# JosephCatrambone/aruco3

Hardware: AMD Instinct MI355X
Metric: frames/sec at 1920x1080 ARUCO dict (higher is better)
Workload: dtype u8

## Files before the change

aruco3_amd/_lib.py:

```python
import ctypes as C
from pathlib import Path

import numpy as np

import os

_HERE = Path(__file__).resolve().parent
LIB_PATH = Path(os.environ["A3_HIP_LIB"]).resolve() if os.environ.get("A3_HIP_LIB") else _HERE / "libaruco3_hip.so"

OK, ERR_INVALID, ERR_HIP, ERR_CAPACITY, ERR_INTERNAL, ERR_NO_DEVICE, ERR_LIMIT = 0, -1, -2, -3, -4, -5, -6
FMT_RGB8, FMT_RGBA8, FMT_L8, FMT_BGRA8 = 0, 1, 2, 3
MEM_HOST, MEM_DEVICE = 0, 1
PROFILE_OFF, PROFILE_STAGES, PROFILE_THRESHOLD_ONLY, PROFILE_THRESHOLD_SAMPLED = 0, 1, 2, 3
STAGE_THRESHOLD, STAGE_CONTOUR, STAGE_DECODE = 0, 1, 2
STEP_WHOLE, STEP_DECODE_DEFERRED, STEP_HELD_RELEASED_BY_LAST, STEP_HELD_RELEASED_EARLY, STEP_BURST_LAST, STEP_HELD = 0, 1, 2, 3, 4, 5
REFINE_NONE, REFINE_SUBPIX = 0, 1
BOARD_NONE, BOARD_OK = 0, 1
BOARD_MAX_MARKERS = 1024
DIST_NONE, DIST_RATIONAL = 0, 1
DIST_FISHEYE = 3
CHARUCO_MAX_CORNERS = 2048
CHARUCO_NO_ADJ = 0xFFFFFFFF
CALIB_FIX_PRINCIPAL_POINT, CALIB_ZERO_TANGENT_DIST, CALIB_FIX_K3, CALIB_RATIONAL_MODEL, CALIB_USE_INTRINSIC_GUESS = 1, 2, 4, 8, 16
CALIB_OK, CALIB_TOO_FEW, CALIB_NO_INIT, CALIB_NOT_FINITE = 1, 2, 3, 4
# ... 6 lines not shown
RIG_OBS_USED, RIG_OBS_TOO_FEW_POINTS, RIG_OBS_DEGENERATE = 1, 2, 3
RIG_FRAME_USED, RIG_FRAME_UNUSED = 1, 2
RIG_MAX_CAMERAS, RIG_MAX_FRAMES, RIG_MAX_RIGS, RIG_MAX_CALL_FRAMES, RIG_MAX_CALL_OBSERVATIONS = 8, 4096, 1024, 65536, 262144
HANDEYE_USE_GUESS, HANDEYE_FIX_X = 1, 2
HANDEYE_OK, HANDEYE_TOO_FEW_FRAMES, HANDEYE_NO_MOTION, HANDEYE_NOT_FINITE = 1, 2, 3, 4
HANDEYE_FRAME_USED, HANDEYE_FRAME_TOO_FEW_POINTS, HANDEYE_FRAME_DEGENERATE = 1, 2, 3
HANDEYE_MAX_FRAMES, HANDEYE_MAX_PROBLEMS, HANDEYE_MAX_CALL_FRAMES = 256, 1024, 65536
HANDEYE_MIN_PIVOT_RATIO = 1e-4
MAP_USE_GUESS, MAP_FIX_MAP = 1, 2
MAP_OK, MAP_NOT_CONNECTED, MAP_NOT_FINITE = 1, 2, 3
MAP_MARKER_USED, MAP_MARKER_UNSEEN, MAP_MARKER_UNREACHED = 1, 2, 3
MAP_FRAME_USED, MAP_FRAME_UNUSED = 1, 2
MAP_OBS_USED, MAP_OBS_DEGENERATE, MAP_OBS_UNREACHED = 1, 2, 3
MAP_MAX_MARKERS, MAP_MAX_FRAMES, MAP_MAX_MAPS, MAP_MAX_CALL_FRAMES, MAP_MAX_CALL_OBSERVATIONS, MAP_START_OBSERVATIONS = 128, 4096, 1024, 65536, 262144, 8
STEP_NAMES = {0: "whole", 1: "decode_deferred", 2: "held_released_by_last", 3: "held_released_early", 4: "burst_last", 5: "held"}

SYMBOLS = [
    "a3_abi_version", "a3_default_config", "a3_create", "a3_destroy", "a3_last_error", "a3_set_stream", "a3_get_stream", "a3_set_pool_limits",
    "a3_get_tau", "a3_order_after", "a3_set_debug_taps", "a3_detect_batch", "a3_detect_batch_pose", "a3_detect_batch_submit", "a3_detect_batch_collect", "a3_detect_batch_pose_submit", "a3_detect_batch_pose_collect",
    "a3_host_alloc", "a3_host_free", "a3_host_register", "a3_host_unregister", "a3_get_stats", "a3_synth_render", "a3_download_grey", "a3_download_thresholded",
    "a3_candidate_count", "a3_download_candidates", "a3_download_homographies", "a3_estimate_pose", "a3_estimate_pose_normalized",
    "a3_find_nearest", "a3_calculate_tau", "a3_set_profiling", "a3_get_profile",
    "a3_contour_count", "a3_download_contours", "a3_detection_record_bytes", "a3_pack_detections",
    "a3_default_refine_config", "a3_set_corner_refinement", "a3_get_refined_corners", "a3_refine_corners",
    "a3_set_board", "a3_get_board_poses", "a3_estimate_board_pose",
    "a3_default_recover_config", "a3_set_board_recovery", "a3_get_board_recovery", "a3_get_recovered_counts", "a3_recover_markers",
    "a3_default_distortion", "a3_set_distortion", "a3_get_undistorted_corners", "a3_undistort_points",
    "a3_default_charuco_config", "a3_set_charuco", "a3_get_charuco_corners", "a3_get_charuco_poses", "a3_interpolate_charuco",
    "a3_calibrate_cameras", "a3_calibrate_fisheye_cameras", "a3_calibrate_rigs", "a3_calibrate_hand_eyes", "a3_build_marker_maps",
    "a3_default_rectify", "a3_rectify_frames", "a3_set_rectification", "a3_get_rectification",
]
CAND_DTYPE = np.dtype([("start_key", "<u4"), ("xy", "<u2", (8,))])
PROJ_DTYPE = np.dtype([("inv", "<f4", (9,)), ("ok", "<i4")])
INTERNAL_SYMBOLS = ["a3_debug_set_overlap", "a3_debug_build_flags", "a3_debug_spin", "a3_debug_set_hold", "a3_debug_set_jump_rounds", "a3_debug_launch_threshold", "a3_debug_kernel_time", "a3_selftest_ieee", "a3_debug_clockwise", "a3_debug_rotate_bits", "a3_debug_discard_too_near", "a3_debug_inject_candidates", "a3_debug_sample_frames", "a3_debug_frame_candidates"]


class A3Error(RuntimeError):
    def __init__(self, code, message):
        super().__init__(f"aruco3_hip error {code}: {message}")
        self.code = code


class Config(C.Structure):
    _fields_ = [
        ("threshold_window", C.c_uint32),
        ("contour_simplification_epsilon", C.c_double),
        ("min_side_length_factor", C.c_float),
        ("min_corner_separation_factor", C.c_float),
        ("homography_sample_size", C.c_uint32),
        ("filter_high_bit_errors", C.c_uint8),
    ]


class MarkerRec(C.Structure):
    _fields_ = [
        ("frame", C.c_uint32),
        ("id", C.c_uint32),
        ("code", C.c_uint64),
        ("corners", C.c_uint32 * 8),
        ("hamming_distance", C.c_uint8),
        ("rotation", C.c_uint8),
        ("candidate_index", C.c_uint16),
    ]


MARKER_DTYPE = np.dtype([("frame", "<u4"), ("id", "<u4"), ("code", "<u8"), ("corners", "<u4", (8,)), ("hamming_distance", "u1"),
                         ("rotation", "u1"), ("candidate_index", "<u2")], align=True)
# ... 359 lines not shown
        L.a3_calibrate_hand_eyes.restype = C.c_int
        L.a3_calibrate_hand_eyes.argtypes = [vp, C.POINTER(HandEyeProblem), C.c_size_t, C.POINTER(HandEyeFrame), C.c_size_t, f32p, f32p,
                                             C.POINTER(HandEyeResult), C.POINTER(HandEyeFrameResult)]
    if hasattr(L, "a3_build_marker_maps"):
        L.a3_build_marker_maps.restype = C.c_int
        L.a3_build_marker_maps.argtypes = [vp, C.POINTER(Map), C.c_size_t, C.POINTER(MapMarker), C.c_size_t, C.POINTER(MapObservation),
                                           C.c_size_t, f32p, C.POINTER(MapResult), C.POINTER(MapMarkerResult), C.POINTER(MapFrame),
                                           C.POINTER(MapObservationResult)]
    if hasattr(L, "a3_calibrate_cameras"):
        L.a3_calibrate_cameras.restype = C.c_int
        L.a3_calibrate_cameras.argtypes = [vp, C.POINTER(CalibCamera), C.c_size_t, u32p, C.c_size_t, f32p, f32p, C.POINTER(CalibResult),
                                           C.POINTER(CalibView)]
    if hasattr(L, "a3_calibrate_fisheye_cameras"):
        L.a3_calibrate_fisheye_cameras.restype = C.c_int
        L.a3_calibrate_fisheye_cameras.argtypes = [vp, C.POINTER(CalibCamera), C.c_size_t, u32p, C.c_size_t, f32p, f32p, C.POINTER(CalibResult),
                                                   C.POINTER(CalibView)]
    if hasattr(L, "a3_rectify_frames"):
        L.a3_default_rectify.restype = None
        L.a3_default_rectify.argtypes = [C.POINTER(RectifyRec), C.POINTER(Intrinsics), C.POINTER(DistortionRec)]
        L.a3_rectify_frames.restype = C.c_int
        L.a3_rectify_frames.argtypes = [vp, vp, C.c_int, C.c_int, C.c_size_t, C.c_size_t, C.c_uint32, C.POINTER(RectifyRec), vp, C.c_int,
                                        C.c_size_t, C.c_size_t, C.POINTER(RectifyInfo)]
    if hasattr(L, "a3_set_rectification"):
        L.a3_set_rectification.restype = C.c_int
        L.a3_set_rectification.argtypes = [vp, C.POINTER(RectifyRec)]
        L.a3_get_rectification.restype = C.c_int
        L.a3_get_rectification.argtypes = [vp, C.POINTER(RectifyRec), C.POINTER(C.c_int)]
    L.a3_debug_discard_too_near.restype = C.c_int
    L.a3_debug_discard_too_near.argtypes = [vp, u32p, C.c_size_t, C.c_float, u32p, C.POINTER(C.c_size_t)]
    if hasattr(L, "a3_debug_frame_candidates"):
        L.a3_debug_frame_candidates.restype = C.c_int
        L.a3_debug_frame_candidates.argtypes = [vp, C.c_uint32, C.c_uint32, u32p, vp, C.c_float, C.c_uint32, C.POINTER(C.c_uint16),
                                                C.POINTER(C.c_uint16), u32p, u32p, u32p, vp]
    _lib = L
    return L


def library_info() -> dict:
    L = load()
    flags = int(L.a3_debug_build_flags()) if hasattr(L, "a3_debug_build_flags") else -1
    return {"path": str(LIB_PATH), "from_A3_HIP_LIB": bool(os.environ.get("A3_HIP_LIB")), "tuning_build": bool(flags & 1) if flags >= 0 else None,
            "non_default_kernel_build": bool(flags & 2) if flags >= 0 else None, "abi": int(L.a3_abi_version())}


class PinnedBuffer:

    def __init__(self, nbytes: int):
        p = C.c_void_p()
        rc = load().a3_host_alloc(nbytes, C.byref(p))
        if rc != OK:
            raise A3Error(rc, load().a3_last_error(None).decode("utf-8", "replace"))
        self.ptr, self.nbytes = p.value, nbytes
        self.array = np.ctypeslib.as_array((C.c_uint8 * nbytes).from_address(p.value))

    def close(self):
        if getattr(self, "ptr", None):
            self.array = None
            load().a3_host_free(C.c_void_p(self.ptr))
            self.ptr = None

    def __del__(self):
        try:
            self.close()
        except Exception:
            pass

# ... 456 lines not shown
    def debug_inject_candidates(self, quads: np.ndarray):
        q = np.ascontiguousarray(quads, dtype=np.uint32).reshape(-1, 8)
        check(load().a3_debug_inject_candidates(self.handle, _p(q, C.c_uint32), q.shape[0]), self)

    def debug_sample_frames(self, on: bool):
        check(load().a3_debug_sample_frames(self.handle, int(on)), self.handle)

    def debug_discard_too_near(self, quads: np.ndarray, min_distance: float) -> np.ndarray:
        q = np.ascontiguousarray(quads, dtype=np.uint32).reshape(-1, 8)
        out = np.zeros_like(q)
        n = C.c_size_t()
        check(load().a3_debug_discard_too_near(self.handle, _p(q, C.c_uint32), q.shape[0], min_distance, _p(out, C.c_uint32), C.byref(n)),
              self.handle)
        return out[: n.value].reshape(-1, 4, 2)

    def debug_frame_candidates(self, cand_count, records: np.ndarray, max_cand: int, min_distance: float, S: int = 0) -> dict:
        cnt = np.ascontiguousarray(cand_count, dtype=np.uint32).reshape(-1)
        rec = np.ascontiguousarray(records, dtype=CAND_DTYPE).reshape(-1)
        n = cnt.shape[0]
        if max_cand >= 1 and rec.shape[0] != int(np.minimum(cnt, max_cand).sum()):
            raise ValueError("records must hold min(cand_count, max_cand) entries per frame")
        slots = n * max_cand if 1 <= max_cand <= 65536 else 0
        pre = np.empty((n, slots // max(n, 1), 8), dtype=np.uint16)
        fin = np.empty_like(pre)
        fin_count = np.empty(n, dtype=np.uint32)
        work = np.empty(slots, dtype=np.uint32)
        work_count = np.zeros(1, dtype=np.uint32)
        proj = np.empty(slots if S else 0, dtype=PROJ_DTYPE)
        check(load().a3_debug_frame_candidates(self.handle, n, max_cand, _p(cnt, C.c_uint32), rec.ctypes.data if rec.size else None, min_distance, S,
                                               _p(pre, C.c_uint16), _p(fin, C.c_uint16), _p(fin_count, C.c_uint32), _p(work, C.c_uint32),
                                               _p(work_count, C.c_uint32), proj.ctypes.data if S else None), self.handle)
        return {"pre_xy": pre, "fin_xy": fin, "fin_count": fin_count, "work": work, "work_count": int(work_count[0]), "proj": proj if S else None}

    def estimate_pose(self, corners: np.ndarray, marker_size_mm: float, image_size=None, intrinsics: Intrinsics = None) -> np.ndarray:
        c = np.ascontiguousarray(corners, dtype=np.uint32).reshape(-1, 8)
        out = (PoseRec * (2 * max(c.shape[0], 1)))()
        iw, ih = image_size if image_size else (1, 1)
        check(load().a3_estimate_pose(self.handle, _p(c, C.c_uint32), c.shape[0], marker_size_mm, C.byref(intrinsics) if intrinsics else None,
                                      iw, ih, out), self.handle)
        return out

    def estimate_pose_normalized(self, points: np.ndarray, marker_size_mm: float):
        p = np.ascontiguousarray(points, dtype=np.float32).reshape(-1, 8)
        out = (PoseRec * (2 * max(p.shape[0], 1)))()
        check(load().a3_estimate_pose_normalized(self.handle, _p(p, C.c_float), p.shape[0], marker_size_mm, out), self.handle)
        return out

    def find_nearest(self, bits: np.ndarray):
        b = np.ascontiguousarray(bits, dtype=np.uint64)
        idx = np.zeros(max(b.size, 1), dtype=np.uint32)
        dist = np.zeros(max(b.size, 1), dtype=np.uint8)
        check(load().a3_find_nearest(self.handle, _p(b, C.c_uint64), b.size, _p(idx, C.c_uint32), _p(dist, C.c_uint8)), self.handle)
        return idx[: b.size], dist[: b.size]

    def selftest_ieee(self, a: np.ndarray, b: np.ndarray):
        a = np.ascontiguousarray(a, dtype=np.float64)
        b = np.ascontiguousarray(b, dtype=np.float64)
        n = a.size
        sq, dv = np.zeros(n), np.zeros(n)
        sqf, dvf = np.zeros(n, dtype=np.float32), np.zeros(n, dtype=np.float32)
        check(load().a3_selftest_ieee(self.handle, _p(a, C.c_double), _p(b, C.c_double), n, _p(sq, C.c_double), _p(dv, C.c_double),
                                      _p(sqf, C.c_float), _p(dvf, C.c_float)), self.handle)
        return sq, dv, sqf, dvf


_dict_ctx = {}
# ... 22 lines not shown
```

aruco3_amd/csrc/a3_api.hip:

```cpp
#include <algorithm>
#include <atomic>
#include <cmath>
#include <chrono>
#include <cstddef>
#include <cstdio>
#include <cstring>
#include <mutex>
#include <string>
#include <vector>

#include "a3_common.h"
#include "a3_internal.h"
#include "a3_launch.h"
#include "a3_readback.h"
#include "a3_rectify_check.h"
#include "a3_solve_check.h"

using namespace a3;

namespace {

thread_local std::string g_create_error;

constexpr uint32_t kPatchCapMin = 32768, kPatchCapMax = 1u << 20;
// ... 1790 lines not shown
    if (int rcs_ = need_stream(ctx)) return rcs_;
    struct Own : DevBuf { ~Own() { release(); } } d_cands, d_cnt, d_pre, d_fin, d_work, d_proj, d_big;
    const bool big = max_cand > frame_cand_lds_slots();
    const size_t proj_bytes = S ? slots * proj_rec_bytes() : 0;
    A3_HIP(d_cands.ensure(slots * sizeof(CandRec)));
    A3_HIP(d_cnt.ensure(((size_t)2 * n_frames + 1) * 4));
    A3_HIP(d_pre.ensure(slots * 16)); A3_HIP(d_fin.ensure(slots * 16)); A3_HIP(d_work.ensure(slots * 4));
    if (S) A3_HIP(d_proj.ensure(proj_bytes));
    if (big) A3_HIP(d_big.ensure(slots * 4));
    uint32_t* cnt = d_cnt.as<uint32_t>();
    hipStream_t st = ctx->stream;
    A3_HIP(hipMemcpyAsync(d_cands.p, h.data(), slots * sizeof(CandRec), hipMemcpyHostToDevice, st));
    A3_HIP(hipMemcpyAsync(cnt, cand_count, (size_t)n_frames * 4, hipMemcpyHostToDevice, st));
    A3_HIP(hipMemsetAsync(cnt + n_frames, 0xFF, (size_t)n_frames * 4, st));
    A3_HIP(hipMemsetAsync(cnt + 2 * (size_t)n_frames, 0, 4, st));
    A3_HIP(hipMemsetAsync(d_pre.p, 0xFF, slots * 16, st)); A3_HIP(hipMemsetAsync(d_fin.p, 0xFF, slots * 16, st));
    A3_HIP(hipMemsetAsync(d_work.p, 0xFF, slots * 4, st));
    if (S) A3_HIP(hipMemsetAsync(d_proj.p, 0xFF, proj_bytes, st));
    if (big) A3_HIP(hipMemsetAsync(d_big.p, 0xFF, slots * 4, st));
    A3_HIP(launch_frame_candidates(st, {.n_frames = n_frames, .max_cand = max_cand, .cands = d_cands.as<CandRec>(), .cand_count = cnt, .min_distance = min_distance,
                                        .pre_xy = d_pre.as<uint16_t>(), .fin_xy = d_fin.as<uint16_t>(), .fin_count = cnt + n_frames, .work = d_work.as<uint32_t>(),
                                        .work_count = cnt + 2 * (size_t)n_frames, .S = S, .proj = S ? d_proj.p : nullptr,
                                        .big_scratch = big ? d_big.as<float>() : nullptr}));
    A3_HIP(hipMemcpyAsync(pre_xy, d_pre.p, slots * 16, hipMemcpyDeviceToHost, st));
    A3_HIP(hipMemcpyAsync(fin_xy, d_fin.p, slots * 16, hipMemcpyDeviceToHost, st));
    A3_HIP(hipMemcpyAsync(fin_count, cnt + n_frames, (size_t)n_frames * 4, hipMemcpyDeviceToHost, st));
    A3_HIP(hipMemcpyAsync(work, d_work.p, slots * 4, hipMemcpyDeviceToHost, st));
    A3_HIP(hipMemcpyAsync(work_count, cnt + 2 * (size_t)n_frames, 4, hipMemcpyDeviceToHost, st));
    if (S) A3_HIP(hipMemcpyAsync(proj, d_proj.p, proj_bytes, hipMemcpyDeviceToHost, st));
    A3_HIP(hipStreamSynchronize(ctx->stream));
    return A3_OK;
}

int a3_debug_inject_candidates(a3_ctx* ctx, const uint32_t* quads_xy, size_t n) {
    if (!ctx || (!quads_xy && n)) return A3_ERR_INVALID;
    if (ctx->batch.active || ctx->pending_trivial) return fail(ctx, A3_ERR_INVALID, "a3_debug_inject_candidates: a submitted batch has not been collected");
    if (n > kMaxCandDefault) return fail(ctx, A3_ERR_CAPACITY, "a3_debug_inject_candidates: at most 1024 quads");
    ctx->inject.resize(n);
    for (size_t i = 0; i < n; i++) {
        ctx->inject[i].start_key = (uint32_t)i;
        for (int k = 0; k < 8; k++) {
            if (quads_xy[8 * i + k] > 65535u) return fail(ctx, A3_ERR_INVALID, "coordinates above 65535");
            ctx->inject[i].xy[k] = (uint16_t)quads_xy[8 * i + k];
        }
    }
    ctx->inject_armed = true;
    return A3_OK;
}

int a3_debug_sample_frames(a3_ctx* ctx, int enabled) {
    if (!ctx) return A3_ERR_INVALID;
    ctx->debug_sample_frames = enabled != 0;
    return A3_OK;
}

void a3_default_refine_config(a3_refine_config* cfg) {
    if (!cfg) return;
    cfg->method = A3_REFINE_SUBPIX; cfg->win_half = 5; cfg->relative_win = 0.4f; cfg->max_iterations = 30; cfg->min_shift = 0.01f;
}

static int check_refine_config(a3_ctx* ctx, const a3_refine_config& c) {
    if (c.method != A3_REFINE_NONE && c.method != A3_REFINE_SUBPIX) return fail(ctx, A3_ERR_INVALID, "a3_refine_config.method: unknown method");
    if (c.method == A3_REFINE_NONE) return A3_OK;
    if (c.win_half < 1 || c.win_half > 10) return fail(ctx, A3_ERR_INVALID, "a3_refine_config.win_half must be in 1..10");
    if (!(c.relative_win >= 0.0f) || !std::isfinite(c.relative_win)) return fail(ctx, A3_ERR_INVALID, "a3_refine_config.relative_win must be finite and >= 0");
    if (c.max_iterations > 100) return fail(ctx, A3_ERR_INVALID, "a3_refine_config.max_iterations must be at most 100");
// ... 690 lines not shown
```

aruco3_amd/csrc/a3_internal.h:

```cpp
#ifndef ARUCO3_HIP_INTERNAL_H
#define ARUCO3_HIP_INTERNAL_H

#include "../../include/aruco3_hip.h"

#ifdef __cplusplus
extern "C" {
#endif

int  a3_debug_kernel_time(a3_ctx *ctx, int kernel, int dbg, int reps, float *avg_ms);

int  a3_debug_set_overlap(int mode);

int  a3_debug_spin(void *hip_stream, int workgroups, int threads, int usec);

int  a3_debug_set_hold(int on);

int  a3_debug_set_jump_rounds(int rounds);

int  a3_debug_launch_threshold(a3_ctx *ctx, const void *pixels_device, int fmt, uint32_t width, uint32_t height, uint32_t n_frames);

int  a3_debug_build_flags(void);

int  a3_selftest_ieee(a3_ctx *ctx, const double *a, const double *b, size_t n, double *sqrt_a, double *a_div_b,
                      float *sqrtf_a, float *a_divf_b);

int  a3_debug_clockwise(a3_ctx *ctx, const int32_t *quads_xy, size_t n, int32_t *out_xy);
int  a3_debug_rotate_bits(a3_ctx *ctx, const uint8_t *bits, uint32_t n, uint32_t times, uint8_t *out);
int  a3_debug_inject_candidates(a3_ctx *ctx, const uint32_t *quads_xy, size_t n);
int  a3_debug_sample_frames(a3_ctx *ctx, int enabled);
int  a3_debug_discard_too_near(a3_ctx *ctx, const uint32_t *quads_xy, size_t n, float min_distance, uint32_t *out_xy, size_t *n_out);

typedef struct { uint32_t start_key; uint16_t xy[8]; } a3_debug_cand;
#define A3_DEBUG_PROJ_BYTES 40
int  a3_debug_frame_candidates(a3_ctx *ctx, uint32_t n_frames, uint32_t max_cand, const uint32_t *cand_count, const a3_debug_cand *records,
                               float min_distance, uint32_t S, uint16_t *pre_xy, uint16_t *fin_xy, uint32_t *fin_count, uint32_t *work,
                               uint32_t *work_count, void *proj);

#ifdef __cplusplus
}
#endif
#endif
```

aruco3_amd/csrc/k_contours.hip:

```cpp
#include <algorithm>
#include <cmath>

#include "a3_common.h"
#include "a3_launch.h"


namespace a3 {

constexpr int kFinB = 8;
constexpr int kScatB = 1;

struct Nb8 { uint64_t c; uint64_t n[8]; };

__device__ __forceinline__ uint64_t ldw(const uint64_t* __restrict__ img, int wpr, int H, int j, int y) {
    return (y >= 0 && y < H && j >= 0 && j < wpr) ? img[(size_t)y * wpr + j] : 0ull;
}

__device__ __forceinline__ void pdart_words(const Nb8& nb, uint64_t p[8]) {
#pragma unroll
    for (int k = 0; k < 8; k++) {
        uint64_t m = nb.c & nb.n[k] & ~nb.n[(k + 7) & 7];
        if ((k & 1) == 0) m &= ~nb.n[(k + 6) & 7];
        p[k] = m;
    }
// ... 1324 lines not shown
    const int dx1 = hq[2] - hq[0], dy1 = hq[3] - hq[1], dx2 = hq[4] - hq[0], dy2 = hq[5] - hq[1];
    if (dx1 * dy2 - dy1 * dx2 < 0) { const int tx = hq[2], ty = hq[3]; hq[2] = hq[6]; hq[3] = hq[7]; hq[6] = tx; hq[7] = ty; }
}

__global__ void k_debug_clockwise(const int32_t* __restrict__ in, uint32_t n, int32_t* __restrict__ out) {
    const uint32_t i = blockIdx.x * blockDim.x + threadIdx.x;
    if (i >= n) return;
    int q[8];
    for (int k = 0; k < 8; k++) q[k] = in[8 * i + k];
    enforce_clockwise(q);
    for (int k = 0; k < 8; k++) out[8 * i + k] = q[k];
}

#define A3_DPP_MAX64(V, CTRL, ROWMASK)                                                                                   \
    {                                                                                                                    \
        const uint32_t lo_ = (uint32_t)__builtin_amdgcn_update_dpp(0, (int)(uint32_t)(V), CTRL, ROWMASK, 0xF, false);        \
        const uint32_t hi_ = (uint32_t)__builtin_amdgcn_update_dpp(0, (int)(uint32_t)((V) >> 32), CTRL, ROWMASK, 0xF, false); \
        const unsigned long long o_ = ((unsigned long long)hi_ << 32) | lo_;                                             \
        (V) = o_ > (V) ? o_ : (V);                                                                                       \
    }
template <int G>
__device__ __forceinline__ unsigned long long group_max_u64(unsigned long long v) {
    A3_DPP_MAX64(v, 0x111, 0xF)
    A3_DPP_MAX64(v, 0x112, 0xF)
    A3_DPP_MAX64(v, 0x114, 0xF)
    A3_DPP_MAX64(v, 0x118, 0xF)
    if constexpr (G == 16) return __shfl(v, 15, 16);
    A3_DPP_MAX64(v, 0x142, 0xA)
    A3_DPP_MAX64(v, 0x143, 0xC)
    const uint32_t lo = (uint32_t)__builtin_amdgcn_readlane((int)(uint32_t)v, 63), hi = (uint32_t)__builtin_amdgcn_readlane((int)(uint32_t)(v >> 32), 63);
    return ((unsigned long long)hi << 32) | lo;
}
#undef A3_DPP_MAX64

constexpr uint32_t kSmallBorder = 64;
template <int G>
__device__ __forceinline__ void contour_quads_body(uint32_t block, uint32_t n_blocks, const ContourRec* __restrict__ contours, const DeviceCounters* __restrict__ ctr,
                                                       uint32_t max_contours, const uint32_t* __restrict__ points, double eps_factor,
                                                       uint32_t min_edge_length, uint32_t first_frame, uint32_t max_cand,
                                                       CandRec* __restrict__ cands, uint32_t* __restrict__ cand_count,
                                                       unsigned int* __restrict__ err_flags, bool coords14) {
    if (ctr->err_flags & (kErrPointPool | kErrContourTable)) return;
    const uint32_t n_contours = min(ctr->contours, max_contours);
    const int lane = threadIdx.x & (G - 1);
    const uint32_t wave_global = (block * blockDim.x + threadIdx.x) / G, n_waves = (n_blocks * blockDim.x) / G;
    for (uint32_t c = wave_global; c < n_contours; c += n_waves) {
        const ContourRec r = contours[c];
        if ((r.n <= kSmallBorder) != (G == 16)) continue;
        const uint32_t* P = points + r.point_base;
        const uint32_t n = r.n;
        const double eps = (double)n * eps_factor;
        uint32_t seg_a[8], seg_b[8];
        int nseg = 1, splits = 0;
        uint32_t kept[3];
        seg_a[0] = 0; seg_b[0] = n - 1;
        bool reject = false;
        while (nseg > 0 && !reject) {
            nseg--;
            const uint32_t a = seg_a[nseg], b = seg_b[nseg];
            const uint32_t pa = P[a], pb = P[b];
            const int ax = pa & 0xFFFF, ay = pa >> 16, bx = pb & 0xFFFF, by = pb >> 16;
            const int la = ay - by, lb = bx - ax;
            const long long lc = (long long)ax * by - (long long)bx * ay;
            unsigned long long best = 0;
            for (uint32_t i0 = a + 1 + lane; i0 <= b; i0 += 4 * G) {
                uint32_t p[4];
#pragma unroll
                for (int u = 0; u < 4; u++) p[u] = P[min(i0 + (uint32_t)u * G, b)];
#pragma unroll
                for (int u = 0; u < 4; u++) {
                    const uint32_t i = i0 + (uint32_t)u * G;
                    if (i > b) break;
                    unsigned long long anum;
                    if (coords14) {
                        const int v = __mul24(la, (int)(p[u] & 0xFFFF)) + __mul24(lb, (int)(p[u] >> 16)) + (int)lc;
                        anum = (unsigned long long)(uint32_t)(v < 0 ? -v : v);
                    } else {
                        long long num = (long long)la * (int)(p[u] & 0xFFFF) + (long long)lb * (int)(p[u] >> 16) + lc;
                        anum = (unsigned long long)(num < 0 ? -num : num);
                    }
                    const unsigned long long cand = (anum << 30) | (unsigned long long)(~i & 0x3FFFFFFFu);
                    if (cand > best) best = cand;
                }
            }
            best = group_max_u64<G>(best);
            const unsigned long long num = best >> 30;
            if (num == 0) continue;
            const uint32_t index = ~(uint32_t)best & 0x3FFFFFFFu;
            const double dn = (double)num, den = (double)((long long)la * la + (long long)lb * lb);
            const double lhs = dn * dn, rhs = eps * eps * den;
            bool far;
            if (lhs > rhs * (1.0 + 1e-9)) far = true;
            else if (lhs < rhs * (1.0 - 1e-9)) far = false;
            else far = dn / sqrt(den) > eps;
            if (far) {
                if (splits == 3) { reject = true; break; }
                kept[splits++] = index;
                seg_a[nseg] = a; seg_b[nseg] = index; nseg++;
                seg_a[nseg] = index; seg_b[nseg] = b; nseg++;
            }
        }
        if (reject || splits != 3) continue;
        if (lane != 0) continue;
        uint32_t k0 = kept[0], k1 = kept[1], k2 = kept[2], t;
        if (k0 > k1) { t = k0; k0 = k1; k1 = t; }
        if (k1 > k2) { t = k1; k1 = k2; k2 = t; }
        if (k0 > k1) { t = k0; k0 = k1; k1 = t; }
        const uint32_t idx[4] = {0u, k0, k1, k2};
        int q[8], hq[8];
        for (int i = 0; i < 4; i++) { const uint32_t p = P[idx[i]]; q[2 * i] = p & 0xFFFF; q[2 * i + 1] = p >> 16; }
        if (!hull4(q, hq)) continue;
        uint32_t cmin = min_edge_length + 1u;
        for (int i = 0; i < 4; i++) {
            const int j = (i + 1) & 3;
            const int dx = hq[2 * i] - hq[2 * j], dy = hq[2 * i + 1] - hq[2 * j + 1];
            const uint32_t d2 = (uint32_t)(dx * dx + dy * dy);
            cmin = d2 < cmin ? d2 : cmin;
        }
        if (cmin < min_edge_length) continue;
        enforce_clockwise(hq);
        const uint32_t fl = r.frame - first_frame;
        const uint32_t slot = atomicAdd(&cand_count[fl], 1u);
        if (slot >= max_cand) { atomicOr(err_flags, kErrCandTable); continue; }
        CandRec cr;
        cr.start_key = r.start_key;
        for (int i = 0; i < 8; i++) cr.xy[i] = (uint16_t)hq[i];
        cands[(size_t)fl * max_cand + slot] = cr;
    }
}

__global__ __launch_bounds__(256) void k_contour_quads(uint32_t blocks64, const ContourRec* __restrict__ contours, const DeviceCounters* __restrict__ ctr,
                                                       uint32_t max_contours, const uint32_t* __restrict__ points, double eps_factor,
                                                       uint32_t min_edge_length, uint32_t first_frame, uint32_t max_cand,
                                                       CandRec* __restrict__ cands, uint32_t* __restrict__ cand_count,
                                                       unsigned int* __restrict__ err_flags, int coords14) {
    if (blockIdx.x < blocks64)
        contour_quads_body<64>(blockIdx.x, blocks64, contours, ctr, max_contours, points, eps_factor, min_edge_length, first_frame, max_cand, cands,
                               cand_count, err_flags, coords14 != 0);
    else
        contour_quads_body<16>(blockIdx.x - blocks64, gridDim.x - blocks64, contours, ctr, max_contours, points, eps_factor, min_edge_length,
                               first_frame, max_cand, cands, cand_count, err_flags, coords14 != 0);
}

__global__ void k_unpack_bits(const uint64_t* __restrict__ bits, int W, int H, uint8_t* __restrict__ out) {
    const int x = blockIdx.x * blockDim.x + threadIdx.x, y = blockIdx.y;
    if (x >= W) return;
    const int wpr = (int)words_per_row((uint32_t)W);
    out[(size_t)y * W + x] = ((bits[(size_t)y * wpr + (x >> 6)] >> (x & 63)) & 1ull) ? 255 : 0;
}

constexpr int kFinBlocks = 1536;
static inline int blocks_for(uint64_t n, int per_block, int cap) {
    uint64_t b = (n + per_block - 1) / per_block;
    if (b < 1) b = 1;
    if (b > (uint64_t)cap) b = cap;
    return (int)b;
}

__global__ __launch_bounds__(256) void k_zero(uint4* __restrict__ p, uint32_t n16) {
    for (uint32_t i = blockIdx.x * blockDim.x + threadIdx.x; i < n16; i += gridDim.x * blockDim.x) p[i] = make_uint4(0u, 0u, 0u, 0u);
}
hipError_t launch_zero(hipStream_t st, void* p, size_t bytes) {
    const uint32_t n16 = (uint32_t)(bytes / 16);
    hipLaunchKernelGGL(k_zero, dim3(blocks_for(n16, 256, 256)), dim3(256), 0, st, reinterpret_cast<uint4*>(p), n16);
    return hipGetLastError();
}

static size_t tile_off_offset(uint32_t W, uint32_t H, uint32_t n_frames) { return (size_t)dart_tiles(W, H) * n_frames; }
static size_t tile_mask_offset_bytes(uint32_t W, uint32_t H, uint32_t n_frames) { return ((size_t)dart_tiles(W, H) * n_frames * 4 * (1 + kCountHalves) + 7) & ~(size_t)7; }
size_t tile_darts_bytes(uint32_t W, uint32_t H, uint32_t n_frames) { return tile_mask_offset_bytes(W, H, n_frames) + (size_t)dart_tiles(W, H) * n_frames * kCountHalves * 8; }

hipError_t launch_dart_count(hipStream_t st, const DartCountLaunch& d) {
    const uint64_t* const bits = d.bits; const int W = d.W, H = d.H; const uint32_t first_frame = d.first_frame, n_frames = d.n_frames;
    unsigned long long* const frame_darts = d.frame_darts; uint32_t* const tile_darts = d.tile_darts; PlanWords* const plan = d.plan;
// ... 139 lines not shown
```

Measured before the change: 382,800.

## Stage contour points in LDS and use packed dot for Douglas-Peucker quad fitting

```diff
diff --git a/aruco3_amd/_lib.py b/aruco3_amd/_lib.py
--- a/aruco3_amd/_lib.py
+++ b/aruco3_amd/_lib.py
@@ -62,7 +62,7 @@
 ]
 CAND_DTYPE = np.dtype([("start_key", "<u4"), ("xy", "<u2", (8,))])
 PROJ_DTYPE = np.dtype([("inv", "<f4", (9,)), ("ok", "<i4")])
-INTERNAL_SYMBOLS = ["a3_debug_set_overlap", "a3_debug_build_flags", "a3_debug_spin", "a3_debug_set_hold", "a3_debug_set_jump_rounds", "a3_debug_launch_threshold", "a3_debug_kernel_time", "a3_selftest_ieee", "a3_debug_clockwise", "a3_debug_rotate_bits", "a3_debug_discard_too_near", "a3_debug_inject_candidates", "a3_debug_sample_frames", "a3_debug_frame_candidates"]
+INTERNAL_SYMBOLS = ["a3_debug_set_overlap", "a3_debug_build_flags", "a3_debug_spin", "a3_debug_set_hold", "a3_debug_set_jump_rounds", "a3_debug_launch_threshold", "a3_debug_kernel_time", "a3_selftest_ieee", "a3_debug_clockwise", "a3_debug_rotate_bits", "a3_debug_discard_too_near", "a3_debug_inject_candidates", "a3_debug_sample_frames", "a3_debug_frame_candidates", "a3_debug_contour_quads"]
 
 
 class A3Error(RuntimeError):
@@ -488,6 +488,10 @@
         L.a3_debug_frame_candidates.restype = C.c_int
         L.a3_debug_frame_candidates.argtypes = [vp, C.c_uint32, C.c_uint32, u32p, vp, C.c_float, C.c_uint32, C.POINTER(C.c_uint16),
                                                 C.POINTER(C.c_uint16), u32p, u32p, u32p, vp]
+    if hasattr(L, "a3_debug_contour_quads"):
+        L.a3_debug_contour_quads.restype = C.c_int
+        L.a3_debug_contour_quads.argtypes = [vp, C.c_uint32, C.c_uint32, C.c_uint32, u32p, u32p, u32p, C.c_double, C.c_uint32, C.c_uint32,
+                                             u32p, vp, u32p]
     _lib = L
     return L
 
@@ -1010,6 +1014,24 @@
                                                _p(work_count, C.c_uint32), proj.ctypes.data if S else None), self.handle)
         return {"pre_xy": pre, "fin_xy": fin, "fin_count": fin_count, "work": work, "work_count": int(work_count[0]), "proj": proj if S else None}
 
+    def debug_contour_quads(self, size, borders, eps_factor: float, min_edge_length: int, max_cand: int = 1024) -> dict:
+        per_frame = np.array([len(f) for f in borders], dtype=np.uint32)
+        flat = [np.asarray(b, dtype=np.int64).reshape(-1, 2) for f in borders for b in f]
+        lengths = np.array([b.shape[0] for b in flat], dtype=np.uint32)
+        pts = np.concatenate(flat) if flat else np.zeros((0, 2), dtype=np.int64)
+        if pts.size and (pts.min() < 0 or pts.max() > 65535):
+            raise ValueError("coordinates must be in 0..65535")
+        words = np.ascontiguousarray(pts[:, 0] | (pts[:, 1] << 16), dtype=np.uint32)
+        n = per_frame.shape[0]
+        slots = n * max_cand if 1 <= max_cand <= 65536 else 0
+        cnt = np.empty(n, dtype=np.uint32)
+        rec = np.empty((n, slots // max(n, 1)), dtype=CAND_DTYPE)
+        err = np.zeros(1, dtype=np.uint32)
+        check(load().a3_debug_contour_quads(self.handle, size[0], size[1], n, _p(per_frame, C.c_uint32), _p(lengths, C.c_uint32),
+                                            _p(words, C.c_uint32), eps_factor, min_edge_length, max_cand, _p(cnt, C.c_uint32),
+                                            rec.ctypes.data if rec.size else None, _p(err, C.c_uint32)), self.handle)
+        return {"cand_count": cnt, "records": [rec[f, : min(int(cnt[f]), max_cand)] for f in range(n)], "err_flags": int(err[0])}
+
     def estimate_pose(self, corners: np.ndarray, marker_size_mm: float, image_size=None, intrinsics: Intrinsics = None) -> np.ndarray:
         c = np.ascontiguousarray(corners, dtype=np.uint32).reshape(-1, 8)
         out = (PoseRec * (2 * max(c.shape[0], 1)))()
diff --git a/aruco3_amd/csrc/a3_api.hip b/aruco3_amd/csrc/a3_api.hip
--- a/aruco3_amd/csrc/a3_api.hip
+++ b/aruco3_amd/csrc/a3_api.hip
@@ -1846,6 +1846,70 @@
     return A3_OK;
 }
 
+int a3_debug_contour_quads(a3_ctx* ctx, uint32_t width, uint32_t height, uint32_t n_frames, const uint32_t* borders_per_frame,
+                           const uint32_t* lengths, const uint32_t* points, double eps_factor, uint32_t min_edge_length, uint32_t max_cand,
+                           uint32_t* cand_count, a3_debug_cand* records, uint32_t* err_flags) {
+    static_assert(sizeof(a3_debug_cand) == sizeof(CandRec), "a3_debug_cand is a CandRec");
+    if (!ctx) return A3_ERR_INVALID;
+    if (ctx->busy()) return fail(ctx, A3_ERR_INVALID, "a3_debug_contour_quads: a submitted batch has not been collected");
+    if (n_frames == 0 || n_frames > (1u << 16)) return fail(ctx, A3_ERR_INVALID, "a3_debug_contour_quads: n_frames must be in 1..65536");
+    if (width == 0 || height == 0 || width > 65536u || height > 65536u)
+        return fail(ctx, A3_ERR_INVALID, "a3_debug_contour_quads: width and height must be in 1..65536");
+    if (max_cand == 0 || max_cand > kMaxCandLimit) return fail(ctx, A3_ERR_INVALID, "a3_debug_contour_quads: max_cand must be in 1..65536");
+    if (!borders_per_frame || !cand_count || !records || !err_flags) return fail(ctx, A3_ERR_INVALID, "a3_debug_contour_quads: a NULL argument");
+    const size_t slots = (size_t)n_frames * max_cand;
+    if (slots > ((size_t)1 << 26)) return fail(ctx, A3_ERR_LIMIT, "a3_debug_contour_quads: more than 2^26 slots");
+    std::vector<ContourRec> recs;
+    uint64_t n_points = 0;
+    for (uint32_t f = 0; f < n_frames; f++) {
+        if (borders_per_frame[f] && (!lengths || !points)) return fail(ctx, A3_ERR_INVALID, "a3_debug_contour_quads: a NULL argument");
+        for (uint32_t k = 0; k < borders_per_frame[f]; k++) {
+            const uint32_t len = lengths[recs.size()];
+            if (len == 0 || len >= (1u << 30)) return fail(ctx, A3_ERR_INVALID, "a3_debug_contour_quads: a border holds 1 .. 2^30 - 1 points");
+            if (recs.size() >= (1u << 24) || n_points + len > (1ull << 28)) return fail(ctx, A3_ERR_LIMIT, "a3_debug_contour_quads: more than 2^24 borders or 2^28 points");
+            recs.push_back(ContourRec{f, (uint32_t)recs.size(), (uint32_t)n_points, len});
+            n_points += len;
+        }
+    }
+    for (uint64_t i = 0; i < n_points; i++)
+        if ((points[i] & 0xFFFFu) >= width || (points[i] >> 16) >= height) return fail(ctx, A3_ERR_INVALID, "a3_debug_contour_quads: a point outside the image");
+    A3_HIP(hipSetDevice(ctx->device));
+    if (int rcs_ = need_stream(ctx)) return rcs_;
+    hipStream_t st = ctx->stream;
+    ctx->contours_valid = false;
+    const uint32_t n_borders = (uint32_t)recs.size();
+    A3_HIP(ctx->contours.ensure(std::max<size_t>(n_borders, 1) * sizeof(ContourRec)));
+    A3_HIP(ctx->points.ensure(std::max<uint64_t>(n_points, 1) * 4));
+    struct Own : DevBuf { ~Own() { release(); } } d_cands, d_small;
+    A3_HIP(d_cands.ensure(slots * sizeof(CandRec)));
+    const size_t cnt_off = (sizeof(DeviceCounters) + 15) & ~(size_t)15, err_off = cnt_off + (((size_t)n_frames * 4 + 15) & ~(size_t)15);
+    A3_HIP(d_small.ensure(err_off + 16));
+    DeviceCounters hc{};
+    hc.contours = n_borders; hc.points = n_points;
+    A3_HIP(hipMemsetAsync(d_small.p, 0, err_off + 16, st));
+    A3_HIP(hipMemcpyAsync(d_small.p, &hc, sizeof hc, hipMemcpyHostToDevice, st));
+    A3_HIP(hipMemsetAsync(d_cands.p, 0xFF, slots * sizeof(CandRec), st));
+    if (n_borders) A3_HIP(hipMemcpyAsync(ctx->contours.p, recs.data(), (size_t)n_borders * sizeof(ContourRec), hipMemcpyHostToDevice, st));
+    if (n_points) A3_HIP(hipMemcpyAsync(ctx->points.p, points, n_points * 4, hipMemcpyHostToDevice, st));
+    ContourChunk cc;
+    cc.first_frame = 0; cc.n_frames = n_frames; cc.batch_frames = n_frames;
+    cc.n_darts = (uint32_t)std::max<uint64_t>(n_points, 1);
+    cc.W = (int)width; cc.H = (int)height;
+    cc.ctr = reinterpret_cast<DeviceCounters*>(d_small.p);
+    cc.contours = ctx->contours.as<ContourRec>(); cc.max_contours = std::max<uint32_t>(n_borders, 1);
+    cc.points = ctx->points.as<uint32_t>(); cc.max_points = std::max<uint64_t>(n_points, 1);
+    cc.eps_factor = eps_factor; cc.min_edge_length = min_edge_length;
+    cc.cands = d_cands.as<CandRec>(); cc.max_cand = max_cand;
+    cc.cand_count = reinterpret_cast<uint32_t*>(d_small.as<uint8_t>() + cnt_off);
+    cc.err_flags = reinterpret_cast<unsigned int*>(d_small.as<uint8_t>() + err_off);
+    A3_HIP(launch_contour_quads(st, cc));
+    A3_HIP(hipMemcpyAsync(cand_count, cc.cand_count, (size_t)n_frames * 4, hipMemcpyDeviceToHost, st));
+    A3_HIP(hipMemcpyAsync(records, d_cands.p, slots * sizeof(CandRec), hipMemcpyDeviceToHost, st));
+    A3_HIP(hipMemcpyAsync(err_flags, cc.err_flags, 4, hipMemcpyDeviceToHost, st));
+    A3_HIP(hipStreamSynchronize(st));
+    return A3_OK;
+}
+
 int a3_debug_inject_candidates(a3_ctx* ctx, const uint32_t* quads_xy, size_t n) {
     if (!ctx || (!quads_xy && n)) return A3_ERR_INVALID;
     if (ctx->batch.active || ctx->pending_trivial) return fail(ctx, A3_ERR_INVALID, "a3_debug_inject_candidates: a submitted batch has not been collected");
diff --git a/aruco3_amd/csrc/a3_internal.h b/aruco3_amd/csrc/a3_internal.h
--- a/aruco3_amd/csrc/a3_internal.h
+++ b/aruco3_amd/csrc/a3_internal.h
@@ -36,6 +36,10 @@
                                float min_distance, uint32_t S, uint16_t *pre_xy, uint16_t *fin_xy, uint32_t *fin_count, uint32_t *work,
                                uint32_t *work_count, void *proj);
 
+int  a3_debug_contour_quads(a3_ctx *ctx, uint32_t width, uint32_t height, uint32_t n_frames, const uint32_t *borders_per_frame,
+                            const uint32_t *lengths, const uint32_t *points, double eps_factor, uint32_t min_edge_length, uint32_t max_cand,
+                            uint32_t *cand_count, a3_debug_cand *records, uint32_t *err_flags);
+
 #ifdef __cplusplus
 }
 #endif
diff --git a/aruco3_amd/csrc/k_contours.hip b/aruco3_amd/csrc/k_contours.hip
--- a/aruco3_amd/csrc/k_contours.hip
+++ b/aruco3_amd/csrc/k_contours.hip
@@ -1380,10 +1380,149 @@
     return ((unsigned long long)hi << 32) | lo;
 }
 #undef A3_DPP_MAX64
+template <int G, bool MAX>
+__device__ __forceinline__ uint32_t group_reduce_u32(uint32_t v) {
+#define A3_DPP_STEP32(CTRL, ROWMASK)                                                                                       \
+    {                                                                                                                    \
+        const uint32_t o_ = (uint32_t)__builtin_amdgcn_update_dpp(MAX ? 0 : -1, (int)v, CTRL, ROWMASK, 0xF, false);        \
+        v = MAX ? max(o_, v) : min(o_, v);                                                                               \
+    }
+    A3_DPP_STEP32(0x111, 0xF) A3_DPP_STEP32(0x112, 0xF) A3_DPP_STEP32(0x114, 0xF) A3_DPP_STEP32(0x118, 0xF)
+    if constexpr (G == 16) return (uint32_t)__shfl((int)v, 15, 16);
+    A3_DPP_STEP32(0x142, 0xA) A3_DPP_STEP32(0x143, 0xC)
+#undef A3_DPP_STEP32
+    return (uint32_t)__builtin_amdgcn_readlane((int)v, 63);
+}
 
 constexpr uint32_t kSmallBorder = 64;
+constexpr uint32_t kQuadSlab = 1536;
+constexpr uint32_t kQuadSlabWords = 4 * kQuadSlab;
+static_assert(16 * kSmallBorder <= kQuadSlabWords, "the sixteen 16-lane groups of a workgroup share the same LDS");
+constexpr int kQuadChords = 8;
+
 template <int G>
-__device__ __forceinline__ void contour_quads_body(uint32_t block, uint32_t n_blocks, const ContourRec* __restrict__ contours, const DeviceCounters* __restrict__ ctr,
+__device__ __forceinline__ uint32_t group_uniform(uint32_t v) {
+    if constexpr (G == 64) return (uint32_t)__builtin_amdgcn_readfirstlane((int)v);
+    else return v;
+}
+
+struct PoolPoints {
+    const uint32_t* __restrict__ p;
+    static constexpr int kDepth = 4;
+    __device__ __forceinline__ uint32_t operator[](uint32_t i) const { return p[i]; }
+};
+struct SlabPoints {
+    const uint32_t* p;
+    static constexpr int kDepth = 1;
+    __device__ __forceinline__ uint32_t operator[](uint32_t i) const { return p[i]; }
+};
+struct LanePoints {
+    uint32_t mine[4];
+    const uint32_t* p;
+    static constexpr int kDepth = 0;
+    __device__ __forceinline__ uint32_t operator[](uint32_t i) const { return p[i]; }
+};
+
+template <int G, typename Src, typename Visit>
+__device__ __forceinline__ void for_chord_points(const Src& src, uint32_t a, uint32_t b, int lane, Visit&& visit) {
+    constexpr int D = Src::kDepth;
+    if constexpr (D == 0) {
+#pragma unroll
+        for (int u = 0; u < 4; u++) {
+            const uint32_t i = (uint32_t)lane + 16u * u;
+            if (i > a && i < b) visit(i, src.mine[u]);
+        }
+    } else if constexpr (D == 1) {
+        uint32_t j = a + 1;
+#pragma unroll 2
+        for (; j + G <= b; j += G) visit(j + lane, src[j + lane]);
+        if (j + lane < b) visit(j + lane, src[j + lane]);
+    } else {
+        for (uint32_t i0 = a + 1 + lane; i0 < b; i0 += D * G) {
+            uint32_t p[D];
+#pragma unroll
+            for (int u = 0; u < D; u++) p[u] = src[min(i0 + (uint32_t)u * G, b)];
+#pragma unroll
+            for (int u = 0; u < D; u++) visit(i0 + (uint32_t)u * G, p[u]);
+        }
+    }
+}
+
+template <int G, typename Src>
+__device__ __forceinline__ uint32_t chord_far_point32(const Src& src, uint32_t a, uint32_t b, int la, int lb, int lc, int lane, uint32_t& index) {
+    typedef short v2i16 __attribute__((ext_vector_type(2)));
+    const uint32_t lab = ((uint32_t)la & 0xFFFFu) | ((uint32_t)lb << 16);
+    uint32_t best = 0, at = 0;
+    for_chord_points<G>(src, a, b, lane, [&](uint32_t i, uint32_t p) {
+        const int v = __builtin_amdgcn_sdot2(__builtin_bit_cast(v2i16, p), __builtin_bit_cast(v2i16, lab), lc, false);
+        const uint32_t av = (uint32_t)max(v, -v);
+        if (av > best) { best = av; at = i; }
+    });
+    const uint32_t most = group_reduce_u32<G, true>(best);
+    index = most ? group_reduce_u32<G, false>(best == most ? at : 0xFFFFFFFFu) : 0u;
+    return most;
+}
+template <int G, typename Src>
+__device__ __forceinline__ unsigned long long chord_far_point64(const Src& src, uint32_t a, uint32_t b, int la, int lb, long long lc, int lane, uint32_t& index) {
+    unsigned long long best = 0;
+    for_chord_points<G>(src, a, b, lane, [&](uint32_t i, uint32_t p) {
+        const long long num = (long long)la * (int)(p & 0xFFFF) + (long long)lb * (int)(p >> 16) + lc;
+        const unsigned long long anum = (unsigned long long)(num < 0 ? -num : num);
+        const unsigned long long cand = (anum << 30) | (unsigned long long)(~i & 0x3FFFFFFFu);
+        if (cand > best) best = cand;
+    });
+    best = group_max_u64<G>(best);
+    index = ~(uint32_t)best & 0x3FFFFFFFu;
+    return best >> 30;
+}
+
+template <int G, typename Src>
+__device__ __forceinline__ bool dp_quad(const Src& src, uint2* chords, uint32_t n, double eps, bool coords14, int lane, uint32_t* corner ) {
+    if (lane == 0) chords[0] = make_uint2(0u, n - 1u);
+    __builtin_amdgcn_fence(__ATOMIC_ACQ_REL, "wavefront");
+    uint32_t head = 0, tail = 1;
+    while (head < tail) {
+        const uint2 ab = chords[head++];
+        const uint32_t a = group_uniform<G>(ab.x), b = group_uniform<G>(ab.y);
+        if (b - a < 2u) continue;
+        const uint32_t pa = src[a], pb = src[b];
+        const int ax = pa & 0xFFFF, ay = pa >> 16, bx = pb & 0xFFFF, by = pb >> 16;
+        const int la = ay - by, lb = bx - ax;
+        uint32_t index;
+        double dn, den;
+        if (coords14) {
+            const uint32_t num = chord_far_point32<G>(src, a, b, la, lb, ax * by - bx * ay, lane, index);
+            if (num == 0) continue;
+            dn = (double)num; den = (double)(la * la + lb * lb);
+        } else {
+            const unsigned long long num = chord_far_point64<G>(src, a, b, la, lb, (long long)ax * by - (long long)bx * ay, lane, index);
+            if (num == 0) continue;
+            dn = (double)num; den = (double)((long long)la * la + (long long)lb * lb);
+        }
+        const double lhs = dn * dn, rhs = eps * eps * den;
+        bool far;
+        if (lhs > rhs * (1.0 + 1e-9)) far = true;
+        else if (lhs < rhs * (1.0 - 1e-9)) far = false;
+        else far = dn / sqrt(den) > eps;
+        if (group_uniform<G>(far ? 1u : 0u)) {
+            if (tail == 7) return false;
+            if (lane == 0) { chords[tail] = make_uint2(a, index); chords[tail + 1] = make_uint2(index, b); }
+            __builtin_amdgcn_fence(__ATOMIC_ACQ_REL, "wavefront");
+            tail += 2;
+        }
+    }
+    if (tail != 7) return false;
+    uint32_t k0 = chords[1].y, k1 = chords[3].y, k2 = chords[5].y, t;
+    if (k0 > k1) { t = k0; k0 = k1; k1 = t; }
+    if (k1 > k2) { t = k1; k1 = k2; k2 = t; }
+    if (k0 > k1) { t = k0; k0 = k1; k1 = t; }
+    corner[0] = src[0]; corner[1] = src[k0]; corner[2] = src[k1]; corner[3] = src[k2];
+    return true;
+}
+
+template <int G>
+__device__ __forceinline__ void contour_quads_body(uint32_t block, uint32_t n_blocks, uint32_t* slabs, uint2* chord_queues,
+                                                       const ContourRec* __restrict__ contours, const DeviceCounters* __restrict__ ctr,
                                                        uint32_t max_contours, const uint32_t* __restrict__ points, double eps_factor,
                                                        uint32_t min_edge_length, uint32_t first_frame, uint32_t max_cand,
                                                        CandRec* __restrict__ cands, uint32_t* __restrict__ cand_count,
@@ -1391,72 +1530,52 @@
     if (ctr->err_flags & (kErrPointPool | kErrContourTable)) return;
     const uint32_t n_contours = min(ctr->contours, max_contours);
     const int lane = threadIdx.x & (G - 1);
-    const uint32_t wave_global = (block * blockDim.x + threadIdx.x) / G, n_waves = (n_blocks * blockDim.x) / G;
+    const uint32_t group = threadIdx.x / G;
+    constexpr uint32_t kSlab = G == 64 ? kQuadSlab : kSmallBorder;
+    uint32_t* const slab = slabs + group * kSlab;
+    uint2* const chords = chord_queues + group * kQuadChords;
+    const uint32_t wave_global = group_uniform<G>((block * blockDim.x + threadIdx.x) / G), n_waves = (n_blocks * blockDim.x) / G;
     for (uint32_t c = wave_global; c < n_contours; c += n_waves) {
         const ContourRec r = contours[c];
         if ((r.n <= kSmallBorder) != (G == 16)) continue;
+        const uint32_t n = r.n;
+        if (n < 5) continue;
         const uint32_t* P = points + r.point_base;
-        const uint32_t n = r.n;
         const double eps = (double)n * eps_factor;
-        uint32_t seg_a[8], seg_b[8];
-        int nseg = 1, splits = 0;
-        uint32_t kept[3];
-        seg_a[0] = 0; seg_b[0] = n - 1;
-        bool reject = false;
-        while (nseg > 0 && !reject) {
-            nseg--;
-            const uint32_t a = seg_a[nseg], b = seg_b[nseg];
-            const uint32_t pa = P[a], pb = P[b];
-            const int ax = pa & 0xFFFF, ay = pa >> 16, bx = pb & 0xFFFF, by = pb >> 16;
-            const int la = ay - by, lb = bx - ax;
-            const long long lc = (long long)ax * by - (long long)bx * ay;
-            unsigned long long best = 0;
-            for (uint32_t i0 = a + 1 + lane; i0 <= b; i0 += 4 * G) {
-                uint32_t p[4];
-#pragma unroll
-                for (int u = 0; u < 4; u++) p[u] = P[min(i0 + (uint32_t)u * G, b)];
-#pragma unroll
-                for (int u = 0; u < 4; u++) {
-                    const uint32_t i = i0 + (uint32_t)u * G;
-                    if (i > b) break;
-                    unsigned long long anum;
-                    if (coords14) {
-                        const int v = __mul24(la, (int)(p[u] & 0xFFFF)) + __mul24(lb, (int)(p[u] >> 16)) + (int)lc;
-                        anum = (unsigned long long)(uint32_t)(v < 0 ? -v : v);
-                    } else {
-                        long long num = (long long)la * (int)(p[u] & 0xFFFF) + (long long)lb * (int)(p[u] >> 16) + lc;
-                        anum = (unsigned long long)(num < 0 ? -num : num);
-                    }
-                    const unsigned long long cand = (anum << 30) | (unsigned long long)(~i & 0x3FFFFFFFu);
-                    if (cand > best) best = cand;
+        uint32_t corner[4];
+        bool quad;
+        if constexpr (G == 16) {
+            LanePoints src;
+            src.p = slab;
+#pragma unroll
+            for (int u = 0; u < 4; u++) src.mine[u] = P[min((uint32_t)lane + 16u * u, n - 1u)];
+#pragma unroll
+            for (int u = 0; u < 4; u++) {
+                const uint32_t i = (uint32_t)lane + 16u * u;
+                if (i < n) slab[i] = src.mine[u];
+            }
+            __builtin_amdgcn_fence(__ATOMIC_ACQ_REL, "wavefront");
+            quad = dp_quad<G>(src, chords, n, eps, coords14, lane, corner);
+        } else if (n <= kSlab) {
+            constexpr int D = 8;
+            for (uint32_t j = 0; j < n; j += D * G) {
+                uint32_t p[D];
+#pragma unroll
+                for (int u = 0; u < D; u++) p[u] = P[min(j + (uint32_t)u * G + lane, n - 1u)];
+#pragma unroll
+                for (int u = 0; u < D; u++) {
+                    const uint32_t i = j + (uint32_t)u * G + lane;
+                    if (i < n) slab[i] = p[u];
                 }
             }
-            best = group_max_u64<G>(best);
-            const unsigned long long num = best >> 30;
-            if (num == 0) continue;
-            const uint32_t index = ~(uint32_t)best & 0x3FFFFFFFu;
-            const double dn = (double)num, den = (double)((long long)la * la + (long long)lb * lb);
-            const double lhs = dn * dn, rhs = eps * eps * den;
-            bool far;
-            if (lhs > rhs * (1.0 + 1e-9)) far = true;
-            else if (lhs < rhs * (1.0 - 1e-9)) far = false;
-            else far = dn / sqrt(den) > eps;
-            if (far) {
-                if (splits == 3) { reject = true; break; }
-                kept[splits++] = index;
-                seg_a[nseg] = a; seg_b[nseg] = index; nseg++;
-                seg_a[nseg] = index; seg_b[nseg] = b; nseg++;
-            }
-        }
-        if (reject || splits != 3) continue;
-        if (lane != 0) continue;
-        uint32_t k0 = kept[0], k1 = kept[1], k2 = kept[2], t;
-        if (k0 > k1) { t = k0; k0 = k1; k1 = t; }
-        if (k1 > k2) { t = k1; k1 = k2; k2 = t; }
-        if (k0 > k1) { t = k0; k0 = k1; k1 = t; }
-        const uint32_t idx[4] = {0u, k0, k1, k2};
+            __builtin_amdgcn_fence(__ATOMIC_ACQ_REL, "wavefront");
+            quad = dp_quad<G>(SlabPoints{slab}, chords, n, eps, coords14, lane, corner);
+        } else {
+            quad = dp_quad<G>(PoolPoints{P}, chords, n, eps, coords14, lane, corner);
+        }
+        if (!quad || lane != 0) continue;
         int q[8], hq[8];
-        for (int i = 0; i < 4; i++) { const uint32_t p = P[idx[i]]; q[2 * i] = p & 0xFFFF; q[2 * i + 1] = p >> 16; }
+        for (int i = 0; i < 4; i++) { q[2 * i] = corner[i] & 0xFFFF; q[2 * i + 1] = corner[i] >> 16; }
         if (!hull4(q, hq)) continue;
         uint32_t cmin = min_edge_length + 1u;
         for (int i = 0; i < 4; i++) {
@@ -1482,12 +1601,14 @@
                                                        uint32_t min_edge_length, uint32_t first_frame, uint32_t max_cand,
                                                        CandRec* __restrict__ cands, uint32_t* __restrict__ cand_count,
                                                        unsigned int* __restrict__ err_flags, int coords14) {
+    __shared__ uint32_t s_slab[kQuadSlabWords];
+    __shared__ uint2 s_chords[(256 / 16) * kQuadChords];
     if (blockIdx.x < blocks64)
-        contour_quads_body<64>(blockIdx.x, blocks64, contours, ctr, max_contours, points, eps_factor, min_edge_length, first_frame, max_cand, cands,
-                               cand_count, err_flags, coords14 != 0);
+        contour_quads_body<64>(blockIdx.x, blocks64, s_slab, s_chords, contours, ctr, max_contours, points, eps_factor, min_edge_length, first_frame,
+                               max_cand, cands, cand_count, err_flags, coords14 != 0);
     else
-        contour_quads_body<16>(blockIdx.x - blocks64, gridDim.x - blocks64, contours, ctr, max_contours, points, eps_factor, min_edge_length,
-                               first_frame, max_cand, cands, cand_count, err_flags, coords14 != 0);
+        contour_quads_body<16>(blockIdx.x - blocks64, gridDim.x - blocks64, s_slab, s_chords, contours, ctr, max_contours, points, eps_factor,
+                               min_edge_length, first_frame, max_cand, cands, cand_count, err_flags, coords14 != 0);
 }
 
 __global__ void k_unpack_bits(const uint64_t* __restrict__ bits, int W, int H, uint8_t* __restrict__ out) {
```

Result: no change. 383,800 (median of 2 runs) (+0.3%).
